# davidcombei/xAI-Audio-Deepfakes

Hardware: AMD Instinct MI355X
Metric: explanations/sec (16 kHz, 4 s clips) (higher is better)
Workload: dtype f32; 1 GPU; BASELINE config 2 extended to the full explanation: batch 64 x 4 s clips, STFT + wav2vec2-base embedder (to hidden layer 9) + logreg + U-Net mask decoder + masked ISTFT x2 + embedder re-forward x2 + LMAC metrics; batch_per_gpu=64, clip_samples=64000, embedder=wav2vec2-base (seeded random weights)

## Files before the change

include/addvisor_hip.h:

```cpp
#ifndef ADDVISOR_HIP_H
#define ADDVISOR_HIP_H

#include <stdint.h>

#ifdef __cplusplus
extern "C" {
#endif

typedef void* advh_stream_t;

enum {
    ADVH_OK = 0,
    ADVH_EINVAL = -1,
    ADVH_ELAUNCH = -2,
    ADVH_ENOTINIT = -3,
    ADVH_EUNSUPPORTED = -4
};

const char* advh_version(void);

int advh_init(void);

int advh_set_option(const char* name, int value);

// ... 121 lines not shown
int advh_pool_logreg_bwd(const float* coef, const float* dlogit, float* dh, void* dh16, int B, int T, int H, advh_stream_t stream);
int advh_w2v2_frontend_bwd_group(const float* wave, int64_t wave_stride, int n_in, int B, int L, const float* w0,
                                 const float* gamma, const float* stats_ws, const float* norm_ws, const float* mr_ws,
                                 const void* dy0, float* part_ws, float* sums_ws, void* dz0, int T0, int P0, int C0,
                                 advh_stream_t stream);
int advh_wave_bwd(const float* g, const float* wave, int64_t wave_stride, int n_in, int B, int L, const float* stats_ws,
                  float* dxhat_ws, float* part_ws, int normalize, float out_scale, float* dx, int64_t dx_stride, int T0, int P0,
                  advh_stream_t stream);
int advh_scale_rows(const float* x, int x_rows, const float* alpha, float* y, int rows, int64_t n, int accumulate,
                    advh_stream_t stream);
int advh_attr_finalize(const float* g, const float* x, float* out, int mode, int64_t total, advh_stream_t stream);
int advh_time_mask(const float* attr, float* mask, float* wave_in, float* wave_out, const float* wave, int B, int64_t n,
                   advh_stream_t stream);

typedef struct advh_path_desc {
    const float* x;
    const float* base;
    const int32_t* bidx;
    int64_t n;
    uint64_t seed;
    int B, S, base_rows;
    int clip_major;
    float sigma;
} advh_path_desc;
int advh_attr_path_points(const advh_path_desc* d, const float* alpha, int64_t row0, int rows, float* out, advh_stream_t stream);
int advh_attr_path_accumulate(const advh_path_desc* d, const float* grad, const float* w, int mode, int64_t row0, int rows,
                              float* total, float* row_sum, advh_stream_t stream);
int advh_philox_normal(uint64_t seed, int64_t row0, int rows, int64_t n, int raw, float* out, advh_stream_t stream);

typedef struct advh_ablation_desc {
    const float* x;
    const float* base;
    const int32_t* mask;
    int64_t n;
    int B, base_rows, mask_rows;
    int mode;
    int win, stride;
    int K;
} advh_ablation_desc;
int advh_ablation_points(const advh_ablation_desc* d, int64_t row0, int rows, float* out, advh_stream_t stream);
int advh_ablation_accumulate(const advh_ablation_desc* d, const float* f0, const float* fk, float* attr, advh_stream_t stream);

int advh_split_overflow(int reset);
int advh_w2v2_frontend_split(const float* wave, int64_t wave_stride, int n_in, int B, int L, const float* w0,
                             const float* bias0, const float* gamma, const float* beta, int mode, int normalize, float* stats_ws,
                             float* norm_ws, float* mr_ws, void* out, int64_t out_lo, int T0, int P0, int C0, advh_stream_t stream);
int advh_layernorm_split(const void* in, int in_is_f32, int64_t in_ld, int64_t in_lo, const void* add_h, int64_t add_ld,
                         int64_t add_lo, const float* gamma, const float* beta, float* out_f, void* out_h, int64_t out_ld,
                         int64_t out_lo, int M, int C, float eps, int gelu, advh_stream_t stream);
int advh_posconv_gather_split(const float* h, void* xg, int64_t xg_lo, int B, int T, int H, int G, int K, int pad_left,
                              advh_stream_t stream);
int advh_attention_split(const void* qkv, int64_t qkv_lo, void* ctx, int64_t ctx_lo, int B, int T, int H, int heads,
                         advh_stream_t stream);
int advh_unet_stem_split(const float* mag, int Fq, int Tq, int B, int H, int W, const float* wgt, const float* bias,
                         void* out, int64_t out_lo, int PH, int PW, float slope, advh_stream_t stream);
int advh_unet_pack_x_split(const float* mag, int Fq, int Tq, int B, int H, int W, void* cat, int64_t cat_lo, int C, int c0,
                           int PH, int PW, advh_stream_t stream);
int advh_unet_head_split(const void* y, int64_t y_lo, int B, int H, int W, int PH, int PW, const float* wgt, float bias,
                         float* mask, float* logits, advh_stream_t stream);
int advh_layernorm_bwd_split(const void* x, int x_is_f32, int64_t x_lo, const void* dy, int dy_is_f32, int64_t dy_lo,
                             const float* gamma, const float* beta, int gelu_fwd, const float* add, const void* dact_src,
                             int64_t dact_lo, float* out_f, void* out_h, int64_t out_lo, int M, int C, float eps, int remap_T,
                             int remap_P, advh_stream_t stream);
int advh_attention_bwd_split(const void* qkv, int64_t qkv_lo, const void* dctx, int64_t dctx_lo, void* dqkv, int64_t dqkv_lo,
                             int B, int T, int H, int heads, advh_stream_t stream);
int advh_pool_logreg_bwd_split(const float* coef, const float* dlogit, float* dh, void* dh16, int64_t dh16_lo, int B, int T, int H,
                               advh_stream_t stream);
int advh_split_f32(const float* src, void* dst, int64_t dst_lo, int64_t n, advh_stream_t stream);
int advh_posconv_gather_bwd_split(const float* dh, void* xg, int64_t xg_lo, int B, int T, int H, int G, int K, int pad_left,
                                  const void* dact_src, int64_t dact_lo, advh_stream_t stream);
int advh_w2v2_frontend_bwd_group_split(const float* wave, int64_t wave_stride, int n_in, int B, int L, const float* w0,
                                       const float* gamma, const float* stats_ws, const float* norm_ws, const float* mr_ws,
                                       const void* dy0, int64_t dy_lo, float* part_ws, float* sums_ws, void* dz0, int64_t dz_lo,
                                       int T0, int P0, int C0, advh_stream_t stream);
typedef struct advh_resblock_x3_desc {
    const void* X;
    const void* W1;
    const float* b1;
    const void* W2;
    const float* b2;
    void* out_h;
    int M, Wg, w0, w1, k, dil;
    float slope;
    int64_t x_lo, o_lo, w_lo;
} advh_resblock_x3_desc;
int advh_resblock_pair_x3_lds_bytes(int C, int k, int dil);
int advh_resblock_pair_x3(const advh_resblock_x3_desc* d, int C, advh_stream_t stream);
int advh_hifigan_pack_mel_split(const float* mel, void* out, int64_t out_lo, int B, int C, int T, int pad, int halo,
                                advh_stream_t stream);
int advh_hifigan_mrf_mix_split(const void* a, const void* b, const void* c, void* y, float slope, int64_t numel, int64_t lo,
                               advh_stream_t stream);
int advh_hifigan_conv_post_split(const void* x, int64_t x_lo, const float* w, float bias, float* wav, int B, int C, int T, int halo,
                                 int k, advh_stream_t stream);

typedef struct advh_taps_desc {
    const void* X;
    const void* W;
    const float* bias;
    const void* resid;
    void* out_h;
    void* out_h2;
    int M, Hg, Wg, h0, h1, w0, w1;
    int ntap;
    int toff[16];
    int act;
    float slope, slope2;
// ... 119 lines not shown
```

xai-audio-deepfakes_amd/addvisor_hip/_lib.py:

```python
from __future__ import annotations

import ctypes as C
import os
import subprocess

_HERE = os.path.dirname(os.path.abspath(__file__))
LIB_PATH = os.environ.get("ADDVISOR_HIP_LIB") or os.path.join(_HERE, "libaddvisor_hip.so")
CSRC = os.path.join(os.path.dirname(_HERE), "csrc")

ERRORS = {-1: "ADVH_EINVAL (bad argument)", -2: "ADVH_ELAUNCH (HIP launch failed)",
          -3: "ADVH_ENOTINIT (advh_init not called)", -4: "ADVH_EUNSUPPORTED"}


class AdvhError(RuntimeError):
    pass


def build(verbose: bool = False) -> str:
    r = subprocess.run(["make", "-C", CSRC, "-j8"], capture_output=True, text=True)
    if r.returncode != 0:
        raise AdvhError("building libaddvisor_hip.so failed:\n" + r.stdout[-4000:] + r.stderr[-4000:])
    if verbose:
        print(r.stdout)
    return LIB_PATH
# ... 26 lines not shown
    "advh_hifigan_mrf_mix": (_i, [_p, _p, _p, _p, _f, _i64, _p]),
    "advh_hifigan_conv_post": (_i, [_p, _p, _f, _p, _i, _i, _i, _i, _i, _p]),
    "advh_mel_log": (_i, [_p, _p, _p, _i, _i, _i, _i, _p]),
    "advh_layernorm_bwd": (_i, [_p, _i, _p, _i, _p, _p, _i, _p, _p, _p, _p, _i, _i, _f, _i, _i, _p]),
    "advh_attention_bwd_f16": (_i, [_p, _p, _p, _i, _i, _i, _i, _p]),
    "advh_pool_logreg_bwd": (_i, [_p, _p, _p, _p, _i, _i, _i, _p]),
    "advh_w2v2_frontend_bwd_group": (_i, [_p, _i64, _i, _i, _i, _p, _p, _p, _p, _p, _p, _p, _p, _p, _i, _i, _i, _p]),
    "advh_wave_bwd": (_i, [_p, _p, _i64, _i, _i, _i, _p, _p, _p, _i, _f, _p, _i64, _i, _i, _p]),
    "advh_scale_rows": (_i, [_p, _i, _p, _p, _i, _i64, _i, _p]),
    "advh_attr_finalize": (_i, [_p, _p, _p, _i, _i64, _p]),
    "advh_time_mask": (_i, [_p, _p, _p, _p, _p, _i, _i64, _p]),
    "advh_attr_path_points": (_i, [_p, _p, _i64, _i, _p, _p]),
    "advh_attr_path_accumulate": (_i, [_p, _p, _p, _i, _i64, _i, _p, _p, _p]),
    "advh_philox_normal": (_i, [C.c_uint64, _i64, _i, _i64, _i, _p, _p]),
    "advh_ablation_points": (_i, [_p, _i64, _i, _p, _p]),
    "advh_ablation_accumulate": (_i, [_p, _p, _p, _p, _p]),
    "advh_istft_masked_bwd": (_i, [_p, _i64, _p, _p, _p, _i, _i, _i, _i, _p, _i, _i, _i, _i, _i, _p, _p]),
    "advh_istft_bandswap": (_i, [_p, _p, _i, _i, _i, _p, _i64, _i64, _i, _i, _i, _i, _i, _p, _p]),
    "advh_bn_partial_count": (_i, []),
    "advh_bn_stats": (_i, [_p, _p, _p, _p, _p]),
    "advh_bn_coef": (_i, [_p, _p, _p, _i, _f, _f, _f, _p, _p, _p, _p, _p]),
    "advh_bn_bwd_coef": (_i, [_p, _p, _i, _f, _f, _p, _p, _p, _p]),
    "advh_bn_apply": (_i, [_p, _p, _p, _f, _p, _p]),
    "advh_bn_bwd_sums": (_i, [_p, _p, _i, _p, _p, _f, _p, _p, _p]),
    "advh_bn_bwd_apply": (_i, [_p, _p, _i, _p, _p, _p, _f, _p, _i64, _i64, _i64, _i64, _p]),
    "advh_transpose_gather": (_i, [_p, _p, _p, _p]),
    "advh_split_f32": (_i, [_p, _p, _i64, _i64, _p]),
    "advh_unet_head_bwd": (_i, [_p, _p, _p, _f, _i64, _p, _p, _i, _p]),
    "advh_unet_head_wgrad": (_i, [_p, _p, _i64, _p, _p, _p]),
    "advh_unet_stem_wgrad": (_i, [_p, _i, _i, _i, _i, _i, _p, _i, _i, _p, _p, _p]),
    "advh_conv_wgrad2d_parts": (_i, [_i, _i, _i, _i]),
    "advh_conv_wgrad2d_f16": (_i, [_p, _i, _p, _p]),
    "advh_conv_wgrad2d_split_parts": (_i, [_i, _i, _i, _i, _i]),
    "advh_conv_wgrad2d_split": (_i, [_p, _i, _i, _i, _i, _i, _i, _i64, _i64, _p, _p]),
    "advh_resblock_pair_lds_bytes": (_i, [_i, _i, _i]),
    "advh_resblock_pair_f16": (_i, [_p, _i, _p]),
    "advh_conv_taps_tile": (_i, [_i, _i, _i]),
    "advh_conv_taps_lds_bytes": (_i, [_i, _i, _i]),
    "advh_conv_taps_f16": (_i, [_p, _i, _p]),
    "advh_conv_taps_split_tile": (_i, [_i, _i, _i]),
    "advh_conv_taps_split": (_i, [_p, _i, _i64, _i64, _i64, _i64, _p]),
    "advh_conv_taps2d_f16": (_i, [_p, _i, _p]),
    "advh_conv_taps2d_split_lds_bytes": (_i, [_i]),
    "advh_conv_taps2d_split": (_i, [_p, _i, _i64, _i64, _i64, _p]),
    "advh_upconv21_tile_f16": (_i, [_p, _p]),
    "advh_posconv_tile_f16": (_i, [_p, _p]),
    "advh_conv53s21_tile_f16": (_i, [_p, _p]),
    "advh_conv53s21_tile_lds_bytes": (_i, []),
    "advh_posconv_tile_lds_bytes": (_i, [_i, _i]),
    "advh_w2v2_frontend_split": (_i, [_p, _i64, _i, _i, _i, _p, _p, _p, _p, _i, _i, _p, _p, _p, _p, _i64, _i, _i, _i, _p]),
    "advh_layernorm_split": (_i, [_p, _i, _i64, _i64, _p, _i64, _i64, _p, _p, _p, _p, _i64, _i64, _i, _i, _f, _i, _p]),
    "advh_posconv_gather_split": (_i, [_p, _p, _i64, _i, _i, _i, _i, _i, _i, _p]),
    "advh_attention_split": (_i, [_p, _i64, _p, _i64, _i, _i, _i, _i, _p]),
    "advh_unet_stem_split": (_i, [_p, _i, _i, _i, _i, _i, _p, _p, _p, _i64, _i, _i, _f, _p]),
    "advh_unet_pack_x_split": (_i, [_p, _i, _i, _i, _i, _i, _p, _i64, _i, _i, _i, _i, _p]),
    "advh_hifigan_pack_mel_split": (_i, [_p, _p, _i64, _i, _i, _i, _i, _i, _p]),
    "advh_hifigan_mrf_mix_split": (_i, [_p, _p, _p, _p, _f, _i64, _i64, _p]),
    "advh_hifigan_conv_post_split": (_i, [_p, _i64, _p, _f, _p, _i, _i, _i, _i, _i, _p]),
    "advh_unet_head_split": (_i, [_p, _i64, _i, _i, _i, _i, _i, _p, _f, _p, _p, _p]),
    "advh_upconv21_tile_lds_bytes": (_i, []),
    "advh_bn_stats_split": (_i, [_p, _i64, _p, _p, _p, _p]),
    "advh_bn_apply_split": (_i, [_p, _i64, _p, _p, _f, _p, _i64, _p]),
    "advh_bn_bwd_sums_split": (_i, [_p, _i64, _p, _i64, _p, _p, _f, _p, _p, _p]),
    "advh_bn_bwd_apply_split": (_i, [_p, _i64, _p, _i64, _p, _p, _p, _f, _p, _i64, _i64, _i64, _i64, _i64, _p]),
    "advh_unet_head_bwd_split": (_i, [_p, _p, _p, _f, _i64, _p, _p, _i64, _p]),
    "advh_unet_head_wgrad_split": (_i, [_p, _p, _i64, _i64, _p, _p, _p]),
    "advh_unet_stem_wgrad_split": (_i, [_p, _i64, _i, _i, _i, _i, _i, _p, _i, _i, _p, _p, _p]),
    "advh_unet_skip_wgrad": (_i, [_p, _i, _i, _i, _i, _i, _p, _i, _i, _p, _p, _p]),
    "advh_unet_skip_wgrad_split": (_i, [_p, _i64, _i, _i, _i, _i, _i, _p, _i, _i, _p, _p, _p]),
    "advh_split_overflow": (_i, [_i]),
    "advh_resblock_pair_x3_lds_bytes": (_i, [_i, _i, _i]),
    "advh_resblock_pair_x3": (_i, [_p, _i, _p]),
    "advh_layernorm_bwd_split": (_i, [_p, _i, _i64, _p, _i, _i64, _p, _p, _i, _p, _p, _i64, _p, _p, _i64, _i, _i, _f, _i, _i, _p]),
    "advh_attention_bwd_split": (_i, [_p, _i64, _p, _i64, _p, _i64, _i, _i, _i, _i, _p]),
    "advh_pool_logreg_bwd_split": (_i, [_p, _p, _p, _p, _i64, _i, _i, _i, _p]),
    "advh_posconv_gather_bwd_split": (_i, [_p, _p, _i64, _i, _i, _i, _i, _i, _i, _p, _i64, _p]),
    "advh_w2v2_frontend_bwd_group_split": (_i, [_p, _i64, _i, _i, _i, _p, _p, _p, _p, _p, _p, _i64, _p, _p, _p, _i64, _i, _i, _i, _p]),
}

_lib = None


def lib() -> C.CDLL:
    global _lib
    if _lib is None:
        import torch
        if not os.path.exists(LIB_PATH):
            raise AdvhError(f"{LIB_PATH} is missing: run `python -c 'import __graft_entry__ as g; g.build()'` "
                            "(there is no fallback path)")
        l = C.CDLL(LIB_PATH)
        for name, (res, args) in SIGNATURES.items():
            fn = getattr(l, name)
            fn.restype, fn.argtypes = res, args
        _lib = l
    return _lib


class SplitRangeError(AdvhError, FloatingPointError):
    """A kernel of the fp32-class mode met a value outside the split format's range (|x| > 65504)."""


def check_overflow(what: str = "") -> None:
    if _lib is not None and _lib.advh_split_overflow(1):
        raise SplitRangeError((what + ": " if what else "") + "a value left the fp32-class format's range (|x| > 65504 between two "
                              "matrix products): the split planes saturated.  Scale the input / weights, or run precision='f16' "
                              "diagnostics; the reference's fp32 has no such limit (include/addvisor_hip.h, advh_split_overflow)")
# ... 18 lines not shown
```

xai-audio-deepfakes_amd/addvisor_hip/embedder.py:

```python
from __future__ import annotations

import ctypes
import os
from typing import Dict, List, Optional, Tuple

import numpy as np
import torch

from . import _lib, gemm as G
from .synthetic import EmbedderConfig

FE_SLACK_ROWS = 4
BRANCH_F16 = os.environ.get("ADDVISOR_BRANCH_F16", "1") != "0"
POSCONV_TILE = os.environ.get("ADDVISOR_POSCONV_TILE", "1") != "0"


class PosconvDesc(ctypes.Structure):
    _fields_ = [("xg", ctypes.c_void_p), ("W", ctypes.c_void_p), ("bias", ctypes.c_void_p), ("resid", ctypes.c_void_p),
                ("out", ctypes.c_void_p), ("B", ctypes.c_int), ("T", ctypes.c_int), ("H", ctypes.c_int),
                ("G", ctypes.c_int), ("K", ctypes.c_int)]


def _f32(t, dev):
    return t.detach().to(torch.float32).contiguous().to(dev)


def default_precision() -> str:
    p = os.environ.get("ADDVISOR_PRECISION", "f32").lower()
    if p not in ("f16", "f32"):
        raise ValueError("ADDVISOR_PRECISION must be f16 or f32")
    return p


class _LN:
    def __init__(self, sd, prefix, dev):
        self.g, self.b = _f32(sd[prefix + ".weight"], dev), _f32(sd[prefix + ".bias"], dev)
        self.C = self.g.numel()

    def __call__(self, x: torch.Tensor, M: int, eps: float, out_f=None, out_h=None, gelu=False, add_h=None, split=False):
        C = self.C
        if split:
            in_f32 = x.dtype == torch.float32
            assert add_h is None
            _lib.check(_lib.lib().advh_layernorm_split(
                x.data_ptr(), int(in_f32), C, 0 if in_f32 else x.stride(0), None, C, 0, self.g.data_ptr(), self.b.data_ptr(),
                None if out_f is None else out_f.data_ptr(), None if out_h is None else out_h.data_ptr(), C,
                0 if out_h is None else out_h.stride(0), M, C, eps, int(gelu), torch.cuda.current_stream().cuda_stream),
                "advh_layernorm_split")
            return
        _lib.check(_lib.lib().advh_layernorm_add(
            x.data_ptr(), int(x.dtype == torch.float32), C, None if add_h is None else add_h.data_ptr(), C,
            self.g.data_ptr(), self.b.data_ptr(),
            None if out_f is None else out_f.data_ptr(), None if out_h is None else out_h.data_ptr(), C, M, C,
            eps, int(gelu), torch.cuda.current_stream().cuda_stream), "advh_layernorm_add")


class HipEmbedder:

    def __init__(self, cfg: EmbedderConfig, sd: Dict[str, torch.Tensor], coef, intercept, device, precision: Optional[str] = None):
        _lib.init()
        self.cfg, self.dev = cfg, device
        self.precision = precision or default_precision()
        if self.precision not in ("f16", "f32"):
            raise ValueError("precision must be 'f16' or 'f32'")
        self.split = self.precision == "f32"
        self.sd = {k: v.detach().float() for k, v in sd.items()}
        if cfg.conv_kernel[0] != 10 or cfg.conv_stride[0] != 5:
# ... 150 lines not shown
        eps = cfg.layer_norm_eps
        C = cfg.conv_dim
        a, bbuf = ws["fe"]
        mode = 1 if self.layer_mode else 0
        ln0 = self.fe_ln[0]
        sp = self.split
        if sp:
            _lib.check(lib.advh_w2v2_frontend_split(
                wave.data_ptr(), wave.stride(0), n_in, B, L, self.w0.data_ptr(),
                None if self.b0 is None else self.b0.data_ptr(), ln0.g.data_ptr(), ln0.b.data_ptr(), mode, int(normalize),
                ws["stats"].data_ptr(), ws["norm"].data_ptr(), ws["mr"].data_ptr(), a.data_ptr(), a.stride(0), Ls[0], P[0], C[0], st),
                "advh_w2v2_frontend_split")
        else:
            _lib.check(lib.advh_w2v2_frontend(
                wave.data_ptr(), wave.stride(0), n_in, B, L, self.w0.data_ptr(),
                None if self.b0 is None else self.b0.data_ptr(), ln0.g.data_ptr(), ln0.b.data_ptr(), mode, int(normalize),
                ws["stats"].data_ptr(), ws["norm"].data_ptr(), ws["mr"].data_ptr(), a.data_ptr(), Ls[0], P[0], C[0], st),
                "advh_w2v2_frontend")
        if self.layer_mode:
            ln0(a, B * P[0], 1e-5, out_h=a, gelu=True, split=sp)
        cur, nxt = a, bbuf
        nfe = len(Ls)
        for i in range(1, nfe):
            last = i == nfe - 1
            dst = ws["feat"] if last else nxt
            ws["fe_plans"][i - 1].run(cur, out_h=dst)
            if self.layer_mode:
                self.fe_ln[i](dst, M if last else B * P[i], 1e-5, out_h=dst, gelu=True, split=sp)
            cur, nxt = dst, cur
        h, h16 = ws["h"], ws["h16"]
        self.fp_ln(ws["feat"], M, eps, out_h=ws["featn"], split=sp)
        ws["proj"].run(ws["featn"], out_f=h)
        K, Gp = cfg.num_conv_pos_embeddings, cfg.num_conv_pos_embedding_groups
        if sp:
            _lib.check(lib.advh_posconv_gather_split(h.data_ptr(), ws["xg"].data_ptr(), ws["xg"].stride(0), B, T, H, Gp, K, K // 2, st),
                       "advh_posconv_gather_split")
        else:
            _lib.check(lib.advh_posconv_gather(h.data_ptr(), ws["xg"].data_ptr(), B, T, H, Gp, K, K // 2, None, st), "advh_posconv_gather")
        if ws["pos_tile"] is not None:
            d = ws["pos_tile"]
            d.xg, d.resid, d.out = ws["xg"].data_ptr(), h.data_ptr(), h.data_ptr()
            _lib.check(lib.advh_posconv_tile_f16(ctypes.byref(d), st), "advh_posconv_tile_f16")
        else:
            ws["pos"].run(ws["xg"], out_f=h, resid=h)
        stable = cfg.do_stable_layer_norm
        if not stable:
            self.enc_ln(h, M, eps, out_f=h, out_h=h16, split=sp)
        for l in range(self.nl):
            lay = ws["layers"][l]
            if stable:
                self.ln1[l](h, M, eps, out_h=h16, split=sp)
            lay["qkv"].run(h16, out_h=ws["qkv"])
            if sp:
                _lib.check(lib.advh_attention_split(ws["qkv"].data_ptr(), ws["qkv"].stride(0), ws["ctx"].data_ptr(), ws["ctx"].stride(0),
                                                    B, T, H, cfg.num_attention_heads, st), "advh_attention_split")
            else:
                _lib.check(lib.advh_attention_f16(ws["qkv"].data_ptr(), ws["ctx"].data_ptr(), B, T, H,
                                                  cfg.num_attention_heads, st), "advh_attention_f16")
            if not stable and BRANCH_F16 and not sp:
                lay["out"].run(ws["ctx"], out_h=ws["br"])
                self.ln1[l](h, M, eps, out_f=h, out_h=h16, add_h=ws["br"])
                lay["ff1"].run(h16, out_h=ws["ffn"])
                lay["ff2"].run(ws["ffn"], out_h=ws["br"])
                self.ln2[l](h, M, eps, out_f=h, out_h=h16, add_h=ws["br"])
                continue
            lay["out"].run(ws["ctx"], out_f=h, resid=h)
            if stable:
                self.ln2[l](h, M, eps, out_h=h16, split=sp)
            else:
                self.ln1[l](h, M, eps, out_f=h, out_h=h16, split=sp)
            lay["ff1"].run(h16, out_h=ws["ffn"])
            lay["ff2"].run(ws["ffn"], out_f=h, resid=h)
            if not stable:
                self.ln2[l](h, M, eps, out_f=h, out_h=h16, split=sp)
        if stable and self.nl == cfg.num_hidden_layers:
            self.enc_ln(h, M, eps, out_f=h)
        _lib.check(lib.advh_pool_logreg(h.data_ptr(), self.coef.data_ptr(), self.intercept, ws["logit"].data_ptr(),
                                        ws["prob"].data_ptr(), None, B, T, H, st), "advh_pool_logreg")
        hid = h.view(B, T, H).clone() if want_hidden else None
        return hid, ws["logit"].clone().view(B, 1), ws["prob"].clone().view(B, 1)
```

xai-audio-deepfakes_amd/addvisor_hip/embedder_grad.py:

```python
from __future__ import annotations

from typing import Dict, Optional, Tuple

import numpy as np
import torch

from . import _lib, gemm as G
from .embedder import FE_SLACK_ROWS, HipEmbedder


def plan_conv1d_dgrad(B: int, P_out: int, weight: torch.Tensor, stride: int, device=None, cache=None, split: bool = False) -> G.GemmPlan:
    Cout, Cin, k = weight.shape
    s = stride
    nt = -(-k // s)
    assert Cout % 8 == 0 and Cin % 4 == 0
    def w2():
        m = torch.zeros(s * Cin, nt * Cout)
        for phase in range(s):
            for i in range(nt):
                j = phase + s * (nt - 1 - i)
                if j < k:
                    m[phase * Cin:(phase + 1) * Cin, i * Cout:(i + 1) * Cout] = weight[:, :, j].t()
        return m[None]
    cc = Cout // 8
    return G.GemmPlan(M=B * P_out, N=s * Cin, w2=w2, ktab=np.arange(nt * cc, dtype=np.int64),
                      sources=[G.Source(P_out * cc, 0, cc, 0)], Hg=1, Wg=P_out, window=(0, 1, 0, P_out), halo_zero=False,
                      out=(P_out * s * Cin, 0, s * Cin, 0), device=device, cache=cache, split=split), nt


class EmbedderGrad:
    def __init__(self, emb: HipEmbedder, precision: Optional[str] = None):
        if precision not in (None, "f16", "f32"):
            raise ValueError("precision must be None, 'f16' or 'f32'")
        if precision == "f16":
            emb = emb.f16_twin()
        elif precision == "f32" and not emb.split:
            raise ValueError("an fp32-class gradient chain needs an fp32-class embedder (HipEmbedder(precision='f32'))")
        self.emb = emb
        self.split = emb.split
        self.precision = emb.precision
        self.cfg, self.dev, self.sd = emb.cfg, emb.dev, emb.sd
        self.layer_mode = emb.layer_mode
        self.stable = self.cfg.do_stable_layer_norm
        self._ws: Dict[Tuple[int, int], dict] = {}
        self._wcache: dict = {}

    def _workspace(self, B: int, L: int) -> dict:
        key = (B, L)
        if key in self._ws:
            return self._ws[key]
        emb, cfg, dev, sd, sp = self.emb, self.cfg, self.dev, self.sd, self.split
        f = emb._workspace(B, L)
        Ls, P, T, M = f["Ls"], f["P"], f["T"], f["M"]
        for i in range(len(Ls)):
            if P[i] <= Ls[i]:
                raise ValueError("backward needs one zero filler row per clip (P > L)")
        H, I, C = cfg.hidden_size, cfg.intermediate_size, cfg.conv_dim
        nfe, nl = len(Ls), emb.nl
        h16, f32 = torch.float16, torch.float32
        pl = (2,) if sp else ()
        z = lambda *s, dt=h16: torch.zeros(*((pl + tuple(s)) if dt == h16 else s), dtype=dt, device=dev)
# ... 74 lines not shown
        L = n_in if length is None else int(length)
        w = self._workspace(B, L)
        f = w["f"]
        st = torch.cuda.current_stream().cuda_stream
        Ls, P, T, M, H = f["Ls"], f["P"], f["T"], f["M"], cfg.hidden_size
        eps, C, nfe, nl = cfg.layer_norm_eps, cfg.conv_dim, len(f["Ls"]), emb.nl
        ln0 = emb.fe_ln[0]
        lm = self.layer_mode
        body = self._body
        y = [body(t, i) for i, t in enumerate(w["y"])]
        zb = [None if t is None else (body(t, i) if i < nfe - 1 else t) for i, t in enumerate(w["z"])]
        out0 = zb[0] if lm else y[0]
        if sp:
            _lib.check(lib.advh_w2v2_frontend_split(
                wave.data_ptr(), wave.stride(0), n_in, B, L, emb.w0.data_ptr(), None if emb.b0 is None else emb.b0.data_ptr(),
                ln0.g.data_ptr(), ln0.b.data_ptr(), 1 if lm else 0, 1, f["stats"].data_ptr(), f["norm"].data_ptr(), f["mr"].data_ptr(),
                out0.data_ptr(), out0.stride(0), Ls[0], P[0], C[0], st), "advh_w2v2_frontend_split")
        else:
            _lib.check(lib.advh_w2v2_frontend(
                wave.data_ptr(), wave.stride(0), n_in, B, L, emb.w0.data_ptr(), None if emb.b0 is None else emb.b0.data_ptr(),
                ln0.g.data_ptr(), ln0.b.data_ptr(), 1 if lm else 0, 1, f["stats"].data_ptr(), f["norm"].data_ptr(), f["mr"].data_ptr(),
                out0.data_ptr(), Ls[0], P[0], C[0], st), "advh_w2v2_frontend")
        if lm:
            ln0(zb[0], B * P[0], 1e-5, out_h=y[0], gelu=True, split=sp)
        for i in range(1, nfe):
            last = i == nfe - 1
            dst = w["feat"] if last else y[i]
            if lm:
                f["fe_plans"][i - 1].run(y[i - 1], out_h=zb[i])
                emb.fe_ln[i](zb[i], M if last else B * P[i], 1e-5, out_h=dst, gelu=True, split=sp)
            else:
                f["fe_plans"][i - 1].run(y[i - 1], out_h=dst, out_pre=zb[i])
        emb.fp_ln(w["feat"], M, eps, out_h=f["featn"], split=sp)
        h = f["h"]
        f["proj"].run(f["featn"], out_f=h)
        K, Gp = cfg.num_conv_pos_embeddings, cfg.num_conv_pos_embedding_groups
        if sp:
            _lib.check(lib.advh_posconv_gather_split(h.data_ptr(), f["xg"].data_ptr(), f["xg"].stride(0), B, T, H, Gp, K, K // 2, st),
                       "advh_posconv_gather_split")
        else:
            _lib.check(lib.advh_posconv_gather(h.data_ptr(), f["xg"].data_ptr(), B, T, H, Gp, K, K // 2, None, st), "advh_posconv_gather")
        h16 = f["h16"]
        if self.stable:
            f["pos"].run(f["xg"], out_f=w["x"][0], resid=h, out_pre=w["pc"])
        else:
            f["pos"].run(f["xg"], out_f=w["h1"], resid=h, out_pre=w["pc"])
            emb.enc_ln(w["h1"], M, eps, out_f=w["x"][0], out_h=h16, split=sp)
        for l in range(nl):
            lay = f["layers"][l]
            if self.stable:
                emb.ln1[l](w["x"][l], M, eps, out_h=h16, split=sp)
            lay["qkv"].run(h16, out_h=w["qkv"][l])
            if sp:
                _lib.check(lib.advh_attention_split(w["qkv"][l].data_ptr(), w["qkv"][l].stride(0), f["ctx"].data_ptr(), f["ctx"].stride(0),
                                                    B, T, H, cfg.num_attention_heads, st), "advh_attention_split")
            else:
                _lib.check(lib.advh_attention_f16(w["qkv"][l].data_ptr(), f["ctx"].data_ptr(), B, T, H, cfg.num_attention_heads, st),
                           "advh_attention_f16")
            if self.stable:
                lay["out"].run(f["ctx"], out_f=w["m"][l], resid=w["x"][l])
                emb.ln2[l](w["m"][l], M, eps, out_h=h16, split=sp)
                lay["ff1"].run(h16, out_h=f["ffn"], out_pre=w["g1"][l])
                lay["ff2"].run(f["ffn"], out_f=w["x"][l + 1], resid=w["m"][l])
            else:
                lay["out"].run(f["ctx"], out_f=w["s1"][l], resid=w["x"][l])
                emb.ln1[l](w["s1"][l], M, eps, out_f=w["m"][l], out_h=h16, split=sp)
                lay["ff1"].run(h16, out_h=f["ffn"], out_pre=w["g1"][l])
                lay["ff2"].run(f["ffn"], out_f=w["s2"][l], resid=w["m"][l])
                emb.ln2[l](w["s2"][l], M, eps, out_f=w["x"][l + 1], out_h=h16, split=sp)
        final = w["x"][nl]
        self._final_ln = self.stable and nl == cfg.num_hidden_layers
        if self._final_ln:
            emb.enc_ln(w["x"][nl], M, eps, out_f=w["xf"], split=sp)
            final = w["xf"]
        _lib.check(lib.advh_pool_logreg(final.data_ptr(), emb.coef.data_ptr(), emb.intercept, f["logit"].data_ptr(),
                                        f["prob"].data_ptr(), None, B, T, H, st), "advh_pool_logreg")
        self._last = (wave, B, n_in, L)
        return f["logit"].clone().view(B, 1), f["prob"].clone().view(B, 1)

    def _ln_bwd(self, ln, x, dy, M, out_f=None, out_h=None, add=None, dact=None, remap=(0, 0), gelu=False, eps=None):
        eps = self.cfg.layer_norm_eps if eps is None else eps
        st = torch.cuda.current_stream().cuda_stream
        x32, dy32 = int(x.dtype == torch.float32), int(dy.dtype == torch.float32)
        p = lambda t: None if t is None else t.data_ptr()
        if self.split:
            lo = lambda t, is32=0: 0 if (t is None or is32) else t.stride(0)
            _lib.check(_lib.lib().advh_layernorm_bwd_split(
                x.data_ptr(), x32, lo(x, x32), dy.data_ptr(), dy32, lo(dy, dy32), ln.g.data_ptr(), ln.b.data_ptr(), int(gelu), p(add),
                p(dact), lo(dact), p(out_f), p(out_h), lo(out_h), M, ln.C, eps, remap[0], remap[1], st), "advh_layernorm_bwd_split")
            return
        _lib.check(_lib.lib().advh_layernorm_bwd(
            x.data_ptr(), x32, dy.data_ptr(), dy32, ln.g.data_ptr(), ln.b.data_ptr(), int(gelu), p(add), p(dact), p(out_f), p(out_h), M,
            ln.C, eps, remap[0], remap[1], st), "advh_layernorm_bwd")

    def _att_bwd(self, qkv, dctx, dqkv, B, T, H, heads, st):
        lib = _lib.lib()
        if self.split:
            _lib.check(lib.advh_attention_bwd_split(qkv.data_ptr(), qkv.stride(0), dctx.data_ptr(), dctx.stride(0), dqkv.data_ptr(),
                                                    dqkv.stride(0), B, T, H, heads, st), "advh_attention_bwd_split")
        else:
            _lib.check(lib.advh_attention_bwd_f16(qkv.data_ptr(), dctx.data_ptr(), dqkv.data_ptr(), B, T, H, heads, st),
                       "advh_attention_bwd_f16")

    def backward(self, loss_scale: float = 4096.0, seed: Optional[torch.Tensor] = None) -> torch.Tensor:
        emb, cfg, lib, sp = self.emb, self.cfg, _lib.lib(), self.split
        wave, B, n_in, L = self._last
        w = self._workspace(B, L)
        f = w["f"]
# ... 85 lines not shown
```

xai-audio-deepfakes_amd/csrc/attention.hip:

```cpp
#include <hip/hip_runtime.h>
#include <hip/hip_fp16.h>
#include "addvisor_hip.h"
#include "common.h"
#include "device_math.h"

namespace advh {

constexpr float LOG2E = 1.4426950408889634f;

typedef _Float16 f16x8 __attribute__((ext_vector_type(8)));
typedef _Float16 f16x4 __attribute__((ext_vector_type(4)));
typedef float f32x4 __attribute__((ext_vector_type(4)));

template <int NT, int D>
__global__ __launch_bounds__(256, (D <= 64 ? 2 : 1)) void attention_kernel(const _Float16* __restrict__ qkv, _Float16* __restrict__ ctx,
                                                        int T, int H, int dm, float scale) {
    constexpr int NKEY = NT * 16, CH = D / 8, VP = NKEY + 64 , NS = (NT + 1) / 2, KK = D / 32, DT = D / 16;
    __shared__ __attribute__((aligned(16))) _Float16 Ks[NKEY * D];
    __shared__ __attribute__((aligned(16))) _Float16 Vt[D * VP];
    const int tid = threadIdx.x, lane = tid & 63, wv = tid >> 6;
    const int head = blockIdx.x, b = blockIdx.y;
    const long ld = 3L * H;
    const _Float16* base = qkv + (long)b * T * ld + head * dm;
    const int chm = dm / 8;

    constexpr int NIT = (NKEY * CH + 255) / 256;
    f16x8 kreg[NIT], vreg[NIT];
#pragma unroll
    for (int it = 0; it < NIT; ++it) {
        const int i = tid + it * 256, key = i / CH, c = i % CH;
        kreg[it] = f16x8{0, 0, 0, 0, 0, 0, 0, 0};
        vreg[it] = kreg[it];
        if (i < NKEY * CH && key < T && c < chm) {
            kreg[it] = *(const f16x8*)(base + (long)key * ld + H + c * 8);
            vreg[it] = *(const f16x8*)(base + (long)key * ld + 2 * H + c * 8);
        }
    }
#pragma unroll
    for (int it = 0; it < NIT; ++it) {
        const int i = tid + it * 256, key = i / CH, c = i % CH;
        if (i >= NKEY * CH) break;
        *(f16x8*)(Ks + key * D + ((c ^ (key & (CH - 1))) * 8)) = kreg[it];
#pragma unroll
        for (int j = 0; j < 8; ++j) Vt[(c * 8 + j) * VP + (c & 7) * 8 + key] = vreg[it][j];
    }
    __syncthreads();

    const int fr = lane & 15, g = lane >> 4;
    for (int qt = wv; qt * 16 < T; qt += 4) {
        int qrow = qt * 16 + fr;
        int qr = qrow < T ? qrow : T - 1;
        f16x8 qf[KK];
#pragma unroll
        for (int kk = 0; kk < KK; ++kk)
// ... 504 lines not shown
        for (int kt = 0; kt < NT; ++kt)
#pragma unroll
            for (int r = 0; r < 4; ++r) { const float e = exp2f(s[kt][r] - mx); s[kt][r] = e; sum += e; }
        sum += __shfl_xor(sum, 16, 64);
        sum += __shfl_xor(sum, 32, 64);
        const float inv = 1.f / sum;
        f16x8 ph[NS], pl_[NS];
#pragma unroll
        for (int ss = 0; ss < NS; ++ss)
#pragma unroll
            for (int r = 0; r < 4; ++r) {
                _Float16 h0, l0, h1 = (_Float16)0.f, l1 = (_Float16)0.f;
                split_f32_raw(s[2 * ss][r] * inv, h0, l0);
                if (2 * ss + 1 < NT) split_f32_raw(s[(2 * ss + 1 < NT) ? 2 * ss + 1 : 0][r] * inv, h1, l1);
                ph[ss][r] = h0; pl_[ss][r] = l0; ph[ss][4 + r] = h1; pl_[ss][4 + r] = l1;
            }
        f32x4 om[DT], ox[DT];
#pragma unroll
        for (int dt = 0; dt < DT; ++dt) { om[dt] = f32x4{0.f, 0.f, 0.f, 0.f}; ox[dt] = f32x4{0.f, 0.f, 0.f, 0.f}; }
#pragma unroll
        for (int ss = 0; ss < NS; ++ss) {
            const int ra = 32 * ss + 4 * g + q, rb = (2 * ss + 1 < NT) ? ra + 16 : ra;
#pragma unroll
            for (int dt = 0; dt < DT; ++dt) {
                const int chn = dt * 2 + (pp >> 1), sub = (pp & 1) * 8;
                const size_t oa = ((size_t)ra * CH + (chn ^ (ra & 7))) * 16 + sub, ob = ((size_t)rb * CH + (chn ^ (rb & 7))) * 16 + sub;
                trvec h0 = __builtin_amdgcn_ds_read_tr16_b64_v4f16((__attribute__((address_space(3))) trvec*)(vs3 + oa));
                trvec h1 = __builtin_amdgcn_ds_read_tr16_b64_v4f16((__attribute__((address_space(3))) trvec*)(vs3 + ob));
                trvec l0 = __builtin_amdgcn_ds_read_tr16_b64_v4f16((__attribute__((address_space(3))) trvec*)(vs3 + PLB + oa));
                trvec l1 = __builtin_amdgcn_ds_read_tr16_b64_v4f16((__attribute__((address_space(3))) trvec*)(vs3 + PLB + ob));
                f16x8 vh, vl;
                __builtin_memcpy(&vh, &h0, 8);
                __builtin_memcpy((char*)&vh + 8, &h1, 8);
                __builtin_memcpy(&vl, &l0, 8);
                __builtin_memcpy((char*)&vl + 8, &l1, 8);
                ox[dt] = __builtin_amdgcn_mfma_f32_16x16x32_f16(vh, pl_[ss], ox[dt], 0, 0, 0);
                om[dt] = __builtin_amdgcn_mfma_f32_16x16x32_f16(vh, ph[ss], om[dt], 0, 0, 0);
                ox[dt] = __builtin_amdgcn_mfma_f32_16x16x32_f16(vl, ph[ss], ox[dt], 0, 0, 0);
            }
            __builtin_amdgcn_sched_barrier(0);
        }
        if (qrow < T) {
#pragma unroll
            for (int dt = 0; dt < DT; ++dt) {
                float v[4];
#pragma unroll
                for (int r = 0; r < 4; ++r) v[r] = fmaf(ox[dt][r], SPLIT_LO_INV, om[dt][r]);
                store_h_rt<4>(ctx, ((long)b * T + qrow) * H + head * D + dt * 16 + g * 4, ctx_lo, v);
            }
        }
    }
}

}

using namespace advh;

extern "C" int advh_attention_f16(const void* qkv, void* ctx, int B, int T, int H, int heads, advh_stream_t stream) {
    if (!qkv || !ctx || B <= 0 || T <= 0 || heads <= 0 || H % heads) return ADVH_EINVAL;
    const int dm = H / heads;
    if (T > 256 || dm % 8 || dm > 128) return ADVH_EUNSUPPORTED;
    const int D = dm <= 32 ? 32 : (dm <= 64 ? 64 : 128);
    const float scale = 1.f / sqrtf((float)dm);
    dim3 grid(heads, B), block(256);
    hipStream_t s = (hipStream_t)stream;
    const int nt = (T + 15) / 16;
#define ATT(NT_, D_) hipLaunchKernelGGL((attention_kernel<NT_, D_>), grid, block, 0, s, (const _Float16*)qkv, (_Float16*)ctx, T, H, dm, scale)
#define ATT_TR(NT_) hipLaunchKernelGGL((attention_tr_kernel<NT_>), grid, block, 0, s, (const _Float16*)qkv, (_Float16*)ctx, T, H, scale)
    if (dm == 64) {
        if (nt <= 4) ATT_TR(4); else if (nt <= 8) ATT_TR(8); else if (nt <= 13) ATT_TR(13); else ATT_TR(16);
    } else if (D == 64) {
        if (nt <= 4) ATT(4, 64); else if (nt <= 8) ATT(8, 64); else if (nt <= 13) ATT(13, 64); else ATT(16, 64);
    } else if (D == 32) {
        if (nt <= 4) ATT(4, 32); else if (nt <= 8) ATT(8, 32); else if (nt <= 13) ATT(13, 32); else ATT(16, 32);
    } else {
        if (nt <= 4) ATT(4, 128); else if (nt <= 13) ATT(13, 128); else ATT(16, 128);
    }
#undef ATT
#undef ATT_TR
    return ADVH_LAUNCH_CHECK();
}

static size_t att_x3_lds(int nt, int D) { return (size_t)2 * (nt * 16 * D + D * (nt * 16 + 64)) * 2; }

int advh_init_attention() {
#define X3A(NT_, D_)                                                                                                                \
    if (hipFuncSetAttribute((const void*)attention_x3_kernel<NT_, D_>, hipFuncAttributeMaxDynamicSharedMemorySize,                  \
                            (int)att_x3_lds(NT_, D_)) != hipSuccess) return ADVH_ELAUNCH;
    X3A(4, 32) X3A(8, 32) X3A(13, 32) X3A(16, 32) X3A(4, 64) X3A(8, 64) X3A(13, 64) X3A(16, 64)
#undef X3A
#define X3T(NT_)                                                                                                                    \
    if (hipFuncSetAttribute((const void*)attention_x3_tr_kernel<NT_>, hipFuncAttributeMaxDynamicSharedMemorySize, 4 * NT_ * 16 * 64 * 2) != hipSuccess) \
        return ADVH_ELAUNCH;
    X3T(4) X3T(8) X3T(13) X3T(16)
#undef X3T
    if (hipFuncSetAttribute((const void*)attention_x3_stream_kernel<7, 128>, hipFuncAttributeMaxDynamicSharedMemorySize,
                            (int)att_x3_lds(7, 128)) != hipSuccess) return ADVH_ELAUNCH;
    return ADVH_OK;
}

extern "C" int advh_attention_split(const void* qkv, int64_t qkv_lo, void* ctx, int64_t ctx_lo, int B, int T, int H, int heads,
                                    advh_stream_t stream) {
    if (!qkv || !ctx || B <= 0 || T <= 0 || heads <= 0 || H % heads || qkv_lo <= 0 || ctx_lo <= 0 || qkv_lo % 8 || ctx_lo % 4) return ADVH_EINVAL;
    const int dm = H / heads;
    if (T > 256 || dm % 8 || dm > 128) return ADVH_EUNSUPPORTED;
    if (dm > 64) {
        hipLaunchKernelGGL((attention_x3_stream_kernel<7, 128>), dim3(heads, B), dim3(512), att_x3_lds(7, 128), (hipStream_t)stream,
                           (const _Float16*)qkv, (long)qkv_lo, (_Float16*)ctx, (long)ctx_lo, T, H, dm, 1.f / sqrtf((float)dm));
        return ADVH_LAUNCH_CHECK();
    }
    const int D = dm <= 32 ? 32 : 64;
    const float scale = 1.f / sqrtf((float)dm);
    dim3 grid(heads, B);
    hipStream_t s = (hipStream_t)stream;
    const int nt = (T + 15) / 16;
    if (dm == 64) {
#define ATTXT(NT_) hipLaunchKernelGGL((attention_x3_tr_kernel<NT_>), grid, dim3(512), 4 * NT_ * 16 * 64 * 2, s, (const _Float16*)qkv, (long)qkv_lo, (_Float16*)ctx, (long)ctx_lo, T, H, scale)
        if (nt <= 4) ATTXT(4); else if (nt <= 8) ATTXT(8); else if (nt <= 13) ATTXT(13); else ATTXT(16);
#undef ATTXT
        return ADVH_LAUNCH_CHECK();
    }
#define ATTX(NT_, D_) hipLaunchKernelGGL((attention_x3_kernel<NT_, D_>), grid, dim3(512), att_x3_lds(NT_, D_), s, (const _Float16*)qkv, (long)qkv_lo, (_Float16*)ctx, (long)ctx_lo, T, H, dm, scale)
    if (D == 64) { if (nt <= 4) ATTX(4, 64); else if (nt <= 8) ATTX(8, 64); else if (nt <= 13) ATTX(13, 64); else ATTX(16, 64); }
    else { if (nt <= 4) ATTX(4, 32); else if (nt <= 8) ATTX(8, 32); else if (nt <= 13) ATTX(13, 32); else ATTX(16, 32); }
#undef ATTX
    return ADVH_LAUNCH_CHECK();
}

ADVH_SPLIT_FLAG_SETTER(advh_split_flag_attention)
```

Baseline: 1381 explanations/s.

## Add persistent software-pipelined split-f16 attention kernel with triple-buffered LDS staging

Adds a persistent attention kernel for head dim 64 and 129–208 tokens. It launches one block per CU and strides over (batch, head) items. While the current item computes, the next item's K tile and the current V tile are staged asynchronously into a triple-buffered LDS ring, using direct global-to-LDS loads and counted vmcnt waits. The aim is to hide global load latency and cut per-block launch and fill overhead compared with one block per (head, batch). In exchange it adds intricate manual wait and barrier logic, uses a large LDS footprint, and allows only one block per CU. An env flag keeps the old path available.

```diff
diff --git a/include/addvisor_hip.h b/include/addvisor_hip.h
--- a/include/addvisor_hip.h
+++ b/include/addvisor_hip.h
@@ -197,6 +197,8 @@
                               advh_stream_t stream);
 int advh_attention_split(const void* qkv, int64_t qkv_lo, void* ctx, int64_t ctx_lo, int B, int T, int H, int heads,
                          advh_stream_t stream);
+int advh_attention_split_nopipe(const void* qkv, int64_t qkv_lo, void* ctx, int64_t ctx_lo, int B, int T, int H, int heads,
+                                advh_stream_t stream);
 int advh_unet_stem_split(const float* mag, int Fq, int Tq, int B, int H, int W, const float* wgt, const float* bias,
                          void* out, int64_t out_lo, int PH, int PW, float slope, advh_stream_t stream);
 int advh_unet_pack_x_split(const float* mag, int Fq, int Tq, int B, int H, int W, void* cat, int64_t cat_lo, int C, int c0,
diff --git a/xai-audio-deepfakes_amd/addvisor_hip/_lib.py b/xai-audio-deepfakes_amd/addvisor_hip/_lib.py
--- a/xai-audio-deepfakes_amd/addvisor_hip/_lib.py
+++ b/xai-audio-deepfakes_amd/addvisor_hip/_lib.py
@@ -102,6 +102,7 @@
     "advh_layernorm_split": (_i, [_p, _i, _i64, _i64, _p, _i64, _i64, _p, _p, _p, _p, _i64, _i64, _i, _i, _f, _i, _p]),
     "advh_posconv_gather_split": (_i, [_p, _p, _i64, _i, _i, _i, _i, _i, _i, _p]),
     "advh_attention_split": (_i, [_p, _i64, _p, _i64, _i, _i, _i, _i, _p]),
+    "advh_attention_split_nopipe": (_i, [_p, _i64, _p, _i64, _i, _i, _i, _i, _p]),
     "advh_unet_stem_split": (_i, [_p, _i, _i, _i, _i, _i, _p, _p, _p, _i64, _i, _i, _f, _p]),
     "advh_unet_pack_x_split": (_i, [_p, _i, _i, _i, _i, _i, _p, _i64, _i, _i, _i, _i, _p]),
     "advh_hifigan_pack_mel_split": (_i, [_p, _p, _i64, _i, _i, _i, _i, _i, _p]),
diff --git a/xai-audio-deepfakes_amd/addvisor_hip/embedder.py b/xai-audio-deepfakes_amd/addvisor_hip/embedder.py
--- a/xai-audio-deepfakes_amd/addvisor_hip/embedder.py
+++ b/xai-audio-deepfakes_amd/addvisor_hip/embedder.py
@@ -13,6 +13,8 @@
 FE_SLACK_ROWS = 4
 BRANCH_F16 = os.environ.get("ADDVISOR_BRANCH_F16", "1") != "0"
 POSCONV_TILE = os.environ.get("ADDVISOR_POSCONV_TILE", "1") != "0"
+ATTN_PIPE = os.environ.get("ADDVISOR_ATTN_PIPE", "1") != "0"
+ATTN_SPLIT = "advh_attention_split" if ATTN_PIPE else "advh_attention_split_nopipe"
 
 
 class PosconvDesc(ctypes.Structure):
@@ -269,8 +271,8 @@
                 self.ln1[l](h, M, eps, out_h=h16, split=sp)
             lay["qkv"].run(h16, out_h=ws["qkv"])
             if sp:
-                _lib.check(lib.advh_attention_split(ws["qkv"].data_ptr(), ws["qkv"].stride(0), ws["ctx"].data_ptr(), ws["ctx"].stride(0),
-                                                    B, T, H, cfg.num_attention_heads, st), "advh_attention_split")
+                _lib.check(getattr(lib, ATTN_SPLIT)(ws["qkv"].data_ptr(), ws["qkv"].stride(0), ws["ctx"].data_ptr(), ws["ctx"].stride(0),
+                                                    B, T, H, cfg.num_attention_heads, st), ATTN_SPLIT)
             else:
                 _lib.check(lib.advh_attention_f16(ws["qkv"].data_ptr(), ws["ctx"].data_ptr(), B, T, H,
                                                   cfg.num_attention_heads, st), "advh_attention_f16")
diff --git a/xai-audio-deepfakes_amd/addvisor_hip/embedder_grad.py b/xai-audio-deepfakes_amd/addvisor_hip/embedder_grad.py
--- a/xai-audio-deepfakes_amd/addvisor_hip/embedder_grad.py
+++ b/xai-audio-deepfakes_amd/addvisor_hip/embedder_grad.py
@@ -6,7 +6,7 @@
 import torch
 
 from . import _lib, gemm as G
-from .embedder import FE_SLACK_ROWS, HipEmbedder
+from .embedder import ATTN_SPLIT, FE_SLACK_ROWS, HipEmbedder
 
 
 def plan_conv1d_dgrad(B: int, P_out: int, weight: torch.Tensor, stride: int, device=None, cache=None, split: bool = False) -> G.GemmPlan:
@@ -187,8 +187,8 @@
                 emb.ln1[l](w["x"][l], M, eps, out_h=h16, split=sp)
             lay["qkv"].run(h16, out_h=w["qkv"][l])
             if sp:
-                _lib.check(lib.advh_attention_split(w["qkv"][l].data_ptr(), w["qkv"][l].stride(0), f["ctx"].data_ptr(), f["ctx"].stride(0),
-                                                    B, T, H, cfg.num_attention_heads, st), "advh_attention_split")
+                _lib.check(getattr(lib, ATTN_SPLIT)(w["qkv"][l].data_ptr(), w["qkv"][l].stride(0), f["ctx"].data_ptr(), f["ctx"].stride(0),
+                                                    B, T, H, cfg.num_attention_heads, st), ATTN_SPLIT)
             else:
                 _lib.check(lib.advh_attention_f16(w["qkv"][l].data_ptr(), f["ctx"].data_ptr(), B, T, H, cfg.num_attention_heads, st),
                            "advh_attention_f16")
diff --git a/xai-audio-deepfakes_amd/csrc/attention.hip b/xai-audio-deepfakes_amd/csrc/attention.hip
--- a/xai-audio-deepfakes_amd/csrc/attention.hip
+++ b/xai-audio-deepfakes_amd/csrc/attention.hip
@@ -1,5 +1,7 @@
 #include <hip/hip_runtime.h>
 #include <hip/hip_fp16.h>
+#include <algorithm>
+#include <climits>
 #include "addvisor_hip.h"
 #include "common.h"
 #include "device_math.h"
@@ -610,6 +612,202 @@
     }
 }
 
+template <int NT>
+__global__ __launch_bounds__(512, 1) void attention_x3_pipe_kernel(const _Float16* __restrict__ qkv, long qkv_lo, _Float16* __restrict__ ctx,
+                                                                   long ctx_lo, int n_items, int T, int H, int heads, float scale) {
+    constexpr int D = 64, NKEY = NT * 16, CH = 8, NS = (NT + 1) / 2, KK = 2, DT = 4;
+    constexpr int PLB = NKEY * D * 2;
+    constexpr int BUF = 2 * PLB;
+    constexpr int MT = (NT + 7) / 8;
+    constexpr int LPW = 2 * (NKEY * CH / 512);
+    static_assert(LPW >= 2 && LPW <= 62 && NKEY * CH % 64 == 0, "counted vmcnt: whole wave-instructions, 6-bit count");
+    extern __shared__ __attribute__((aligned(16))) _Float16 att_lds[];
+    const int tid = threadIdx.x, lane = tid & 63, wv = tid >> 6;
+    const long ld = 3L * H;
+    const int nqt = (T + 15) / 16;
+    auto fresh = [](int& vl, int& st) { asm volatile("" : "+v"(vl), "+s"(st)); };
+
+    auto stage = [&](int it, int off, char* buf) {
+        const _Float16* base = qkv + (long)(it / heads) * T * ld + (it % heads) * D + off * H;
+        for (int i = tid; i < NKEY * CH; i += 512) {
+            const int key = i / CH, c = (i % CH) ^ (key & 7);
+            const _Float16* src = base + (long)min(key, T - 1) * ld + c * 8;
+            const size_t dst = (size_t)(i - lane) * 16;
+            __builtin_amdgcn_global_load_lds(GLOBAL_PTR(src), LDS_PTR(buf + dst), 16, 0, 0);
+            __builtin_amdgcn_global_load_lds(GLOBAL_PTR(src + qkv_lo), LDS_PTR(buf + PLB + dst), 16, 0, 0);
+        }
+    };
+    f16x8 qh[MT][KK], ql[MT][KK];
+    auto load_q = [&](int it) {
+        int ln = lane, Tq = T;
+        fresh(ln, Tq);
+        const int fr = ln & 15, g = ln >> 4;
+        const _Float16* base = qkv + (long)(it / heads) * T * ld + (it % heads) * D;
+#pragma unroll
+        for (int j = 0; j < MT; ++j) {
+            const int qrow = (wv + 8 * j) * 16 + fr, qr = min(qrow, Tq - 1);
+#pragma unroll
+            for (int kk = 0; kk < KK; ++kk) {
+                qh[j][kk] = *(const f16x8*)(base + (long)qr * ld + kk * 32 + g * 8);
+                ql[j][kk] = *(const f16x8*)(base + qkv_lo + (long)qr * ld + kk * 32 + g * 8);
+            }
+        }
+    };
+    auto q_ready = [&]() {
+#pragma unroll
+        for (int j = 0; j < MT; ++j)
+#pragma unroll
+            for (int kk = 0; kk < KK; ++kk) asm volatile("" ::"v"(qh[j][kk]), "v"(ql[j][kk]));
+    };
+    auto barrier = [&]() {
+        asm volatile("s_waitcnt lgkmcnt(0)" ::: "memory");
+        __builtin_amdgcn_s_barrier();
+        asm volatile("" ::: "memory");
+    };
+
+    char* bk = (char*)att_lds;
+    char* bv = bk + BUF;
+    char* bn = bv + BUF;
+    const int stride = gridDim.x;
+    int it = blockIdx.x;
+    if (it >= n_items) return;
+    stage(it, 1, bk);
+    load_q(it);
+    q_ready();
+    asm volatile("s_waitcnt vmcnt(0)" ::: "memory");
+    barrier();
+
+    for (; it < n_items; it += stride) {
+        const int nx = it + stride;
+        const bool more = nx < n_items;
+        q_ready();
+        stage(it, 2, bv);
+        if (more) stage(nx, 1, bn);
+        const long obase = (long)(it / heads) * T * H + (it % heads) * D;
+
+        f16x8 ph[MT][NS], pl_[MT][NS];
+        int ln = lane, Tq = T;
+        fresh(ln, Tq);
+        const int fr = ln & 15, g = ln >> 4;
+#pragma unroll
+        for (int j = 0; j < MT; ++j) {
+            if ((wv + 8 * j) >= nqt) break;
+            f32x4 s[NT];
+#pragma unroll
+            for (int kt = 0; kt < NT; ++kt) {
+                f32x4 sm = f32x4{0.f, 0.f, 0.f, 0.f}, sx = f32x4{0.f, 0.f, 0.f, 0.f};
+#pragma unroll
+                for (int kk = 0; kk < KK; ++kk) {
+                    const int key = kt * 16 + fr, c = kk * 4 + g;
+                    const int o = (key * CH + (c ^ (key & 7))) * 16;
+                    const f16x8 kh = *(const f16x8*)(bk + o), kl = *(const f16x8*)(bk + PLB + o);
+                    sx = __builtin_amdgcn_mfma_f32_16x16x32_f16(kh, ql[j][kk], sx, 0, 0, 0);
+                    sm = __builtin_amdgcn_mfma_f32_16x16x32_f16(kh, qh[j][kk], sm, 0, 0, 0);
+                    sx = __builtin_amdgcn_mfma_f32_16x16x32_f16(kl, qh[j][kk], sx, 0, 0, 0);
+                }
+#pragma unroll
+                for (int r = 0; r < 4; ++r) s[kt][r] = fmaf(sx[r], SPLIT_LO_INV, sm[r]);
+                if ((kt & 1) == 1) __builtin_amdgcn_sched_barrier(0);
+            }
+            __builtin_amdgcn_sched_barrier(0);
+            int lm = lane, Tm = T;
+            fresh(lm, Tm);
+            const int gm = lm >> 4;
+            float mx = -INFINITY;
+#pragma unroll
+            for (int kt = 0; kt < NT; ++kt)
+#pragma unroll
+                for (int r = 0; r < 4; ++r) {
+                    const float v = (kt * 16 + gm * 4 + r < Tm) ? s[kt][r] * (scale * LOG2E) : -INFINITY;
+                    s[kt][r] = v;
+                    mx = fmaxf(mx, v);
+                }
+            mx = fmaxf(mx, __shfl_xor(mx, 16, 64));
+            mx = fmaxf(mx, __shfl_xor(mx, 32, 64));
+            float sum = 0.f;
+#pragma unroll
+            for (int kt = 0; kt < NT; ++kt)
+#pragma unroll
+                for (int r = 0; r < 4; ++r) { const float e = exp2f(s[kt][r] - mx); s[kt][r] = e; sum += e; }
+            sum += __shfl_xor(sum, 16, 64);
+            sum += __shfl_xor(sum, 32, 64);
+            const float inv = 1.f / sum;
+#pragma unroll
+            for (int ss = 0; ss < NS; ++ss)
+#pragma unroll
+                for (int r = 0; r < 4; ++r) {
+                    _Float16 h0, l0, h1 = (_Float16)0.f, l1 = (_Float16)0.f;
+                    split_f32_raw(s[2 * ss][r] * inv, h0, l0);
+                    if (2 * ss + 1 < NT) split_f32_raw(s[(2 * ss + 1 < NT) ? 2 * ss + 1 : 0][r] * inv, h1, l1);
+                    ph[j][ss][r] = h0; pl_[j][ss][r] = l0; ph[j][ss][4 + r] = h1; pl_[j][ss][4 + r] = l1;
+                }
+        }
+        if (more) asm volatile("s_waitcnt vmcnt(%0)" ::"n"(LPW) : "memory");
+        else asm volatile("s_waitcnt vmcnt(0)" ::: "memory");
+        barrier();
+
+        const auto* vs3 = (const __attribute__((address_space(3))) char*)LDS_PTR(bv);
+        float res[MT][DT][4];
+        ln = lane;
+        Tq = T;
+        fresh(ln, Tq);
+        const int q = (ln >> 2) & 3, pp = ln & 3, gv = ln >> 4, frv = ln & 15;
+#pragma unroll
+        for (int j = 0; j < MT; ++j) {
+            if (j == MT - 1 && more) load_q(nx);
+            if (wv + 8 * j >= nqt) continue;
+            f32x4 om[DT], ox[DT];
+#pragma unroll
+            for (int dt = 0; dt < DT; ++dt) { om[dt] = f32x4{0.f, 0.f, 0.f, 0.f}; ox[dt] = f32x4{0.f, 0.f, 0.f, 0.f}; }
+#pragma unroll
+            for (int ss = 0; ss < NS; ++ss) {
+                const int ra = 32 * ss + 4 * gv + q, rb = (2 * ss + 1 < NT) ? ra + 16 : ra;
+#pragma unroll
+                for (int dt = 0; dt < DT; ++dt) {
+                    const int chn = dt * 2 + (pp >> 1), sub = (pp & 1) * 8;
+                    const size_t oa = ((size_t)ra * CH + (chn ^ (ra & 7))) * 16 + sub, ob = ((size_t)rb * CH + (chn ^ (rb & 7))) * 16 + sub;
+                    trvec h0 = __builtin_amdgcn_ds_read_tr16_b64_v4f16((__attribute__((address_space(3))) trvec*)(vs3 + oa));
+                    trvec h1 = __builtin_amdgcn_ds_read_tr16_b64_v4f16((__attribute__((address_space(3))) trvec*)(vs3 + ob));
+                    trvec l0 = __builtin_amdgcn_ds_read_tr16_b64_v4f16((__attribute__((address_space(3))) trvec*)(vs3 + PLB + oa));
+                    trvec l1 = __builtin_amdgcn_ds_read_tr16_b64_v4f16((__attribute__((address_space(3))) trvec*)(vs3 + PLB + ob));
+                    f16x8 vh, vl;
+                    __builtin_memcpy(&vh, &h0, 8);
+                    __builtin_memcpy((char*)&vh + 8, &h1, 8);
+                    __builtin_memcpy(&vl, &l0, 8);
+                    __builtin_memcpy((char*)&vl + 8, &l1, 8);
+                    ox[dt] = __builtin_amdgcn_mfma_f32_16x16x32_f16(vh, pl_[j][ss], ox[dt], 0, 0, 0);
+                    om[dt] = __builtin_amdgcn_mfma_f32_16x16x32_f16(vh, ph[j][ss], om[dt], 0, 0, 0);
+                    ox[dt] = __builtin_amdgcn_mfma_f32_16x16x32_f16(vl, ph[j][ss], ox[dt], 0, 0, 0);
+                }
+                __builtin_amdgcn_sched_barrier(0);
+            }
+#pragma unroll
+            for (int dt = 0; dt < DT; ++dt)
+#pragma unroll
+                for (int r = 0; r < 4; ++r) res[j][dt][r] = fmaf(ox[dt][r], SPLIT_LO_INV, om[dt][r]);
+        }
+        if (more) {
+            q_ready();
+            asm volatile("s_waitcnt vmcnt(0)" ::: "memory");
+        }
+#pragma unroll
+        for (int j = 0; j < MT; ++j) {
+            const int qrow = (wv + 8 * j) * 16 + frv;
+            if (wv + 8 * j >= nqt) break;
+            if (qrow < Tq) {
+#pragma unroll
+                for (int dt = 0; dt < DT; ++dt) store_h_rt<4>(ctx, obase + (long)qrow * H + dt * 16 + gv * 4, ctx_lo, res[j][dt]);
+            }
+        }
+        if (!more) break;
+        barrier();
+        char* t = bk;
+        bk = bn;
+        bn = bv;
+        bv = t;
+    }
+}
+
 }
 
 using namespace advh;
@@ -640,6 +838,10 @@
 }
 
 static size_t att_x3_lds(int nt, int D) { return (size_t)2 * (nt * 16 * D + D * (nt * 16 + 64)) * 2; }
+static constexpr int att_pipe_lds(int nt) { return 3 * 2 * nt * 16 * 64 * 2; }
+static_assert(att_pipe_lds(13) <= 160 * 1024, "the 13-tile pipeline fits the 160 KB LDS");
+constexpr int ATT_MAX_DEV = 64;
+static int g_att_cus[ATT_MAX_DEV];
 
 int advh_init_attention() {
 #define X3A(NT_, D_)                                                                                                                \
@@ -654,14 +856,35 @@
 #undef X3T
     if (hipFuncSetAttribute((const void*)attention_x3_stream_kernel<7, 128>, hipFuncAttributeMaxDynamicSharedMemorySize,
                             (int)att_x3_lds(7, 128)) != hipSuccess) return ADVH_ELAUNCH;
+#define X3P(NT_)                                                                                                                    \
+    if (hipFuncSetAttribute((const void*)attention_x3_pipe_kernel<NT_>, hipFuncAttributeMaxDynamicSharedMemorySize, att_pipe_lds(NT_)) != hipSuccess) \
+        return ADVH_ELAUNCH;
+    X3P(13)
+#undef X3P
+    int dev = 0, cus = 0;
+    if (hipGetDevice(&dev) != hipSuccess || dev < 0 || dev >= ATT_MAX_DEV) return ADVH_ELAUNCH;
+    if (hipDeviceGetAttribute(&cus, hipDeviceAttributeMultiprocessorCount, dev) != hipSuccess || cus <= 0) return ADVH_ELAUNCH;
+    g_att_cus[dev] = cus;
     return ADVH_OK;
 }
 
-extern "C" int advh_attention_split(const void* qkv, int64_t qkv_lo, void* ctx, int64_t ctx_lo, int B, int T, int H, int heads,
-                                    advh_stream_t stream) {
+static int attention_split(const void* qkv, int64_t qkv_lo, void* ctx, int64_t ctx_lo, int B, int T, int H, int heads,
+                           advh_stream_t stream, bool pipe) {
     if (!qkv || !ctx || B <= 0 || T <= 0 || heads <= 0 || H % heads || qkv_lo <= 0 || ctx_lo <= 0 || qkv_lo % 8 || ctx_lo % 4) return ADVH_EINVAL;
     const int dm = H / heads;
     if (T > 256 || dm % 8 || dm > 128) return ADVH_EUNSUPPORTED;
+    if (pipe && dm == 64 && T > 8 * 16 && T <= 13 * 16) {
+        const long items = (long)B * heads;
+        if (items > INT_MAX) return ADVH_EUNSUPPORTED;
+        int dev = 0;
+        if (hipGetDevice(&dev) != hipSuccess || dev < 0 || dev >= ATT_MAX_DEV || g_att_cus[dev] <= 0) return ADVH_ELAUNCH;
+        const int grid = (int)std::min<long>(items, g_att_cus[dev]);
+#define ATTXP(NT_) hipLaunchKernelGGL((attention_x3_pipe_kernel<NT_>), dim3(grid), dim3(512), att_pipe_lds(NT_), (hipStream_t)stream, \
+                                      (const _Float16*)qkv, (long)qkv_lo, (_Float16*)ctx, (long)ctx_lo, (int)items, T, H, heads, 1.f / sqrtf((float)dm))
+        ATTXP(13);
+#undef ATTXP
+        return ADVH_LAUNCH_CHECK();
+    }
     if (dm > 64) {
         hipLaunchKernelGGL((attention_x3_stream_kernel<7, 128>), dim3(heads, B), dim3(512), att_x3_lds(7, 128), (hipStream_t)stream,
                            (const _Float16*)qkv, (long)qkv_lo, (_Float16*)ctx, (long)ctx_lo, T, H, dm, 1.f / sqrtf((float)dm));
@@ -685,4 +908,14 @@
     return ADVH_LAUNCH_CHECK();
 }
 
+extern "C" int advh_attention_split(const void* qkv, int64_t qkv_lo, void* ctx, int64_t ctx_lo, int B, int T, int H, int heads,
+                                    advh_stream_t stream) {
+    return attention_split(qkv, qkv_lo, ctx, ctx_lo, B, T, H, heads, stream, true);
+}
+
+extern "C" int advh_attention_split_nopipe(const void* qkv, int64_t qkv_lo, void* ctx, int64_t ctx_lo, int B, int T, int H, int heads,
+                                           advh_stream_t stream) {
+    return attention_split(qkv, qkv_lo, ctx, ctx_lo, B, T, H, heads, stream, false);
+}
+
 ADVH_SPLIT_FLAG_SETTER(advh_split_flag_attention)
```

Result: no change. 1385 explanations/s, median of 6 (+0.3%).
